# TritonDataCenter/containerpilot

Hardware: NVIDIA H100
Metric: events/sec through Bus.Publish (deliveries/s = 32-byte records landed in subscriber mailboxes) (higher is better)
Workload: dtype u8

## Files before the change

### containerpilot_b200/csrc/cpbus.cu

```cuda
#include "cpbus_internal.hpp"

#include <algorithm>
#include <chrono>
#include <cstdio>
#include <cstdlib>
#include <cstring>
#include <functional>
#include <mutex>
#include <new>
#include <string>
#include <thread>
#include <unordered_map>
#include <vector>

int cpbus_host::dev_guard(cpbus* b) {
  CK(cudaSetDevice(b->device));
  return CPBUS_OK;
}

static std::chrono::microseconds stream_budget(const cpbus* b) {
  return std::chrono::microseconds(b->stream_spin_us ? b->stream_spin_us : 2000000u);
}

static int stream_error(const cpbus* b) {
// ... 30 lines not shown
    if (f->dbg_head == -1) break;
    const cpbus_event e = f->dbg[f->dbg_tail % 10];
    if (f->dbg_tail == f->dbg_head) { f->dbg_head = -1; f->dbg_tail = 0; }
    else f->dbg_tail = (f->dbg_tail + 1) % 10;
    if (e.code == CPBUS_NONE && e.source_id == 0) break;
    if (k < cap) out[k] = e;
    k++;
  }
  return k;
}

void cpbus_host::dbg_mark_device_batch(HostFront* f, unsigned long long launch) {
  f->dbg_pending.push_back(DbgItem{true, launch, cpbus_event{}});
  if (f->dbg_pending.size() > (size_t)kAcctDbgRing) f->dbg_pending.pop_front();
}

static int rebuild_order(cpbus* b) {
  std::vector<uint32_t> order;
  static_assert(sizeof(b->h_active[0]) == 1, "h_active is a byte vector");
  mask_order(b->h_mask.data(), reinterpret_cast<const uint8_t*>(b->h_active.data()), b->n_next, b->R, b->order_block, true, order);
  b->n_order = (uint32_t)order.size();
  if (b->n_order) {
    CK(cudaMemcpyAsync(b->d_order, order.data(), (size_t)b->n_order * 4, cudaMemcpyHostToDevice, b->stream));
    CK(cudaStreamSynchronize(b->stream));
  }
  b->order_dirty = false;
  return CPBUS_OK;
}

constexpr int kFanoutMaxSmem = 200 * 1024;

enum { kLaunchPlain = 0, kLaunchFollow = 1, kLaunchRound = 2 };

template <int STORE, bool TIMERS, bool DIGEST, bool ORDERED, bool PAIRS = false>
static int launch_fanout_t(cpbus* b, const FanoutParams& p, uint32_t grid, size_t smem, int kind) {
  static bool attr_done[3][64] = {};
  void (*kernel)(FanoutParams) = kind == kLaunchRound  ? fanout_round_kernel<STORE, TIMERS, DIGEST, ORDERED, PAIRS>
                               : kind == kLaunchFollow ? fanout_follow_kernel<STORE, TIMERS, DIGEST, ORDERED, PAIRS>
                                                       : fanout_kernel<STORE, TIMERS, DIGEST, ORDERED, PAIRS>;
  const int dev = b->device & 63;
  if (!attr_done[kind][dev]) {
    CK(cudaFuncSetAttribute(kernel, cudaFuncAttributeMaxDynamicSharedMemorySize, kFanoutMaxSmem));
    attr_done[kind][dev] = true;
  }
  cudaLaunchConfig_t cfg{};
  cfg.gridDim = dim3(grid); cfg.blockDim = dim3(kThreads); cfg.dynamicSmemBytes = smem; cfg.stream = b->stream;
  cudaLaunchAttribute attr[1];
  attr[0].id = cudaLaunchAttributeProgrammaticStreamSerialization;
  attr[0].val.programmaticStreamSerializationAllowed = 1;
  cfg.attrs = attr; cfg.numAttrs = b->pdl && kind != kLaunchRound ? 1 : 0;
  CK(cudaLaunchKernelEx(&cfg, kernel, p));
  CK(cudaGetLastError());
  return CPBUS_OK;
}

template <int ST>
static int preload_round_fanouts() {
  void (*ks[])(FanoutParams) = {
      fanout_round_kernel<ST, false, false, false>, fanout_round_kernel<ST, false, true, false>,
      fanout_round_kernel<ST, true, false, false>, fanout_round_kernel<ST, true, true, false>,
      fanout_round_kernel<ST, false, false, true>, fanout_round_kernel<ST, false, true, true>,
      fanout_round_kernel<ST, true, false, false, true>, fanout_round_kernel<ST, true, true, false, true>};
  for (auto k : ks) CK(cudaFuncSetAttribute(k, cudaFuncAttributeMaxDynamicSharedMemorySize, kFanoutMaxSmem));
  return CPBUS_OK;
}

static int preload_round_kernels(cpbus* b) {
  static bool done[64] = {};
  static std::mutex mu;
  std::lock_guard<std::mutex> g(mu);
  if (done[b->device & 63]) return CPBUS_OK;
  int rc;
  if ((rc = preload_round_fanouts<CPBUS_STORE_V4>()) || (rc = preload_round_fanouts<CPBUS_STORE_V8>()) ||
      (rc = preload_round_fanouts<CPBUS_STORE_BULK>()))
    return rc;
  cudaFuncAttributes a;
  CK(cudaFuncGetAttributes(&a, stream_round_decide_kernel));
  CK(cudaFuncGetAttributes(&a, stream_round_admit_kernel));
  CK(cudaFuncGetAttributes(&a, stream_round_agree_kernel));
  CK(cudaFuncGetAttributes(&a, consume_all_kernel));
  CK(cudaFuncGetAttributes(&a, digest_fold_kernel));
  CK(cudaFuncGetAttributes(&a, blockers_scan_kernel));
  CK(cudaFuncGetAttributes(&a, lagging_scan_kernel));
  done[b->device & 63] = true;
  return CPBUS_OK;
}

struct StreamArgs {
  const StreamHdr* hdr = nullptr; unsigned long long* ack = nullptr; unsigned long long seq = 0;
  const StreamHdr* next_hdr = nullptr;
  uint32_t off = 0; bool final = true;
  FollowRec* follow_rec = nullptr;
  bool follow_from_host = false;
  const RoundDev* round = nullptr;
};
// ... 23 lines not shown
  if (n == 0 && b->n_timers == 0 && !sa) return CPBUS_OK;
  FanoutParams p{};
  p.batch = d_src; p.ring = b->d_ring; p.ctl = b->d_ctl; p.timers = b->d_timers; p.stats = b->d_stats; p.pow_table = b->d_pow; p.launch_seq = ++b->launch_seq;
  p.desc = b->d_desc + (p.launch_seq & 1) * ((fanout_desc_bytes(2048) + 255) & ~(size_t)255);
  p.desc_ready = b->d_desc_ready + (p.launch_seq & 1) * 16; p.w_now = w;
  p.result = result_slot(b, p.launch_seq); p.result_next = result_slot(b, p.launch_seq + 1);
  p.batch_local = b->d_batch_local; p.staged = (uint32_t)o.staged;
  p.err_word = b->h_err.dev(); p.acct = o.account ? b->d_acct.get() : nullptr;
  p.pf_state = b->d_pf_state; p.pf_buf = b->d_pf_buf; p.pf_stride = b->B; p.spin_us = b->stream_spin_us;
  if (sa) {
    p.stream_hdr = sa->hdr; p.stream_ack = sa->ack; p.stream_seq = sa->seq; p.stream_next_hdr = sa->next_hdr;
    p.stream_off = sa->off; p.stream_final = sa->final ? 1u : 0u;
  }
  const bool follow = sa && sa->follow_rec, round = sa && sa->round;
  const int kind = round ? kLaunchRound : follow ? kLaunchFollow : kLaunchPlain;
  p.round = round ? sa->round : nullptr;
  if (follow) {
    p.follow_clock = b->d_follow_clock; p.follow_rec = sa->follow_rec; p.follow_window = max_window(b);
    p.follow_from_host = sa->follow_from_host ? 1u : 0u;
  }
  p.prefetch_src = o.pf_src; p.prefetch_dst = o.pf_dst; p.prefetch_n = o.pf_n;
  p.batch_dep = o.batch_dep ? 1u : 0u; p.n_ev = n;
  p.n_subs = b->n_next; p.ring_cap = b->R; p.K = b->K; p.sub_base = b->cfg.sub_id_base;
  p.use_digest = b->use_digest; p.lossless = b->lossless; p.timers_on = b->n_timers > 0 && b->K > 0;
  p.smem_cap = (n + 31u) & ~31u;
  const size_t hot_bytes = (size_t)b->n_next * (sizeof(SubCtl) + (p.timers_on ? b->K * sizeof(DevTimer) : 0));
  p.hints = b->hints >= 0 ? (uint32_t)b->hints : (hot_bytes <= (64u << 20) ? 1u : 0u);
  const uint32_t need = (b->n_next + kWarpsPerCta - 1) / kWarpsPerCta;
  uint32_t grid = b->cfg.grid_ctas ? std::max(1u, std::min(b->cfg.grid_ctas, need)) : 0u;
  int rc;
  const bool pairs_on = b->n_paired > 0 && b->d_pairs;
  p.pairs = pairs_on ? b->d_pairs.get() : nullptr;
  size_t smem = fanout_smem_bytes(p.smem_cap) + (pairs_on ? kPairFilterBytes : 0);
  if (!pairs_on && !p.timers_on && b->n_filtered > 0) {
    if (b->order_dirty) { const int rc_order = rebuild_order(b); if (rc_order) return rc_order; }
    if (b->n_order) {
      const uint32_t scale = std::max(1u, (p.n_ev + 128u) / 256u);
      uint32_t spw = b->subs_per_warp ? std::min(32u, b->subs_per_warp)
                                      : std::max(4u, std::min(16u / scale, b->n_order / (20480u * scale)));
      p.order = b->d_order; p.n_order = b->n_order; p.spw = spw;
      const uint32_t warps = (b->n_order + spw - 1) / spw;
      grid = std::max(1u, (warps + kWarpsPerCta - 1) / kWarpsPerCta);
    }
  }
  if (pairs_on && !b->cfg.grid_ctas) {
    const uint32_t blocks = (b->n_next + 31u) / 32u;
    grid = std::max(1u, std::min((blocks + kWarpsPerCta - 1) / kWarpsPerCta, (uint32_t)b->sm_count * 16u));
  }
  if (!pairs_on && !p.order) {
    uint32_t spw = b->subs_per_warp;
    if (grid) spw = std::max(1u, (need + grid - 1) / grid);
    else if (!spw) {
      const uint32_t scale = std::max(1u, (p.n_ev + 128u) / 256u);
      const uint32_t cap = std::max(1u, 16u / scale);
      spw = std::max(1u, std::min(cap, (need + (uint32_t)b->sm_count * 7 * scale) / ((uint32_t)b->sm_count * 14 * scale)));
    }
    p.spw = spw;
    grid = std::max(1u, (need + spw - 1) / spw);
    const size_t off = fanout_stage_off(p.smem_cap);
    const size_t per_sub = sizeof(SubCtl) + (p.timers_on ? (size_t)b->K * sizeof(DevTimer) : 0);
    const size_t min_round = (size_t)kWarpsPerCta * per_sub;
    const size_t ctas = std::max<size_t>(1, std::min<size_t>(kCtasPerSm, b->smem_per_sm / (off + min_round + b->smem_reserved)));
    const size_t room = std::min<size_t>(kFanoutMaxSmem, b->smem_per_sm / ctas - b->smem_reserved) - off;
    p.stage_subs = std::max<uint32_t>(kWarpsPerCta, (uint32_t)std::min<size_t>((size_t)kWarpsPerCta * spw, room / per_sub) & ~7u);
    smem = off + p.stage_subs * per_sub;
  }
  const int variant = pairs_on ? (p.use_digest ? 7 : 6) : (p.timers_on ? 2 : 0) | (p.use_digest ? 1 : 0) | (p.order ? 4 : 0);
  std::unique_lock<std::mutex> ready_lock(b->mu, std::defer_lock);
  if (b->sparse_drains) ready_lock.lock();
#define CPBUS_DISPATCH(ST)                                                              \
  switch (variant) {                                                                     \
    case 0: rc = launch_fanout_t<ST, false, false, false>(b, p, grid, smem, kind); break;      \
    case 1: rc = launch_fanout_t<ST, false, true, false>(b, p, grid, smem, kind); break;       \
    case 2: rc = launch_fanout_t<ST, true, false, false>(b, p, grid, smem, kind); break;       \
    case 3: rc = launch_fanout_t<ST, true, true, false>(b, p, grid, smem, kind); break;        \
    case 4: rc = launch_fanout_t<ST, false, false, true>(b, p, grid, smem, kind); break;       \
    case 5: rc = launch_fanout_t<ST, false, true, true>(b, p, grid, smem, kind); break;        \
    case 6: rc = launch_fanout_t<ST, true, false, false, true>(b, p, grid, smem, kind); break; \
    default: rc = launch_fanout_t<ST, true, true, false, true>(b, p, grid, smem, kind); break; \
  }
  switch (b->store) {
    case CPBUS_STORE_V4: CPBUS_DISPATCH(CPBUS_STORE_V4); break;
    case CPBUS_STORE_BULK: CPBUS_DISPATCH(CPBUS_STORE_BULK); break;
    default: CPBUS_DISPATCH(CPBUS_STORE_V8); break;
  }
#undef CPBUS_DISPATCH
  if (b->sparse_drains) b->ready_ix.full();
  if (rc) return rc;
  b->st.kernel_launches++;
  if (!round) b->st.batches++;
  if (sa) return CPBUS_OK;
  launched_to(b, w);
  if (o.account && n) dbg_mark_device_batch(b, p.launch_seq);
  return CPBUS_OK;
}

static void timer_table(cpbus* b) {
  b->h_timers.resize((size_t)b->N * b->K);
  if (b->sparse) b->due.init(b->h_timers.size());
}

static int stage_batch(cpbus* b, uint32_t n, cpbus_event** d_dst) {
  const uint32_t slot = b->dev_slot;
  *d_dst = b->d_stage + (size_t)slot * b->B;
  if (slot % cpbus::kDevEpoch == 0) CK(cudaEventSynchronize(b->epoch_done[slot / cpbus::kDevEpoch]));
  if (n) {
    CK(cudaMemcpyAsync(*d_dst, b->h_batch[b->cur], (size_t)n * sizeof(cpbus_event), cudaMemcpyHostToDevice, b->copy_stream));
    CK(cudaEventRecord(b->h2d_done[b->cur], b->copy_stream));
  }
  return CPBUS_OK;
}

// ... 268 lines not shown
  if ((uint64_t)cfg->sub_id_base + cfg->n_max_subs > CPBUS_TARGET_ALL) return CPBUS_EINVAL;
  *R_out = R; *B_out = B;
  return CPBUS_OK;
}

int cpbus_create(const cpbus_config* cfg, cpbus_t** out) try {
  if (!cfg || !out) return CPBUS_EINVAL;
  *out = nullptr;
  uint32_t R = 0, B = 0;
  if (config_check(cfg, &R, &B)) return CPBUS_EINVAL;
  if ((cfg->flags & CPBUS_CFG_SPARSE_RECORDS) && !(cfg->flags & CPBUS_CFG_SPARSE_TICKS)) return CPBUS_EINVAL;
  if ((cfg->flags & CPBUS_CFG_SPARSE_DRAINS) && !(cfg->flags & CPBUS_CFG_SPARSE_TICKS)) return CPBUS_EINVAL;
  const uint32_t K = cfg->timers_per_sub;
  int ndev = 0;
  if (cudaGetDeviceCount(&ndev) != cudaSuccess || ndev == 0) {
    snprintf(g_cuda_err, sizeof(g_cuda_err), "no CUDA device visible");
    return CPBUS_ENODEV;
  }
  cpbus* b = new (std::nothrow) cpbus();
  if (!b) return CPBUS_ENOMEM;
  b->cfg = *cfg; b->cfg.ring_cap = R; b->cfg.batch_cap = B;
  b->N = cfg->n_max_subs; b->R = R; b->B = B; b->K = K;
  b->lossless = cfg->flags & CPBUS_CFG_LOSSLESS; b->use_digest = cfg->flags & CPBUS_CFG_DIGEST;
  b->sparse = cfg->flags & CPBUS_CFG_SPARSE_TICKS;
  b->sparse_records = cfg->flags & CPBUS_CFG_SPARSE_RECORDS;
  b->sparse_drains = cfg->flags & CPBUS_CFG_SPARSE_DRAINS;
  b->drop_missed = cfg->flags & CPBUS_CFG_DROP_MISSED_TICKS;
  b->room_lb = R;
  b->store = cfg->store_path == CPBUS_STORE_AUTO ? CPBUS_STORE_V8 : (int)cfg->store_path;
  if (const char* e = getenv("CPBUS_PDL")) b->pdl = atoi(e) != 0;
  if (const char* e = getenv("CPBUS_HINTS")) b->hints = atoi(e);
  if (const char* e = getenv("CPBUS_SUBS_PER_WARP")) b->subs_per_warp = (uint32_t)atoi(e);
  if (const char* e = getenv("CPBUS_ORDER_BLOCK")) b->order_block = (uint32_t)atoll(e);
  int rc = CPBUS_OK;
  auto fail = [&](int code) { cpbus_destroy(b); return code; };
  if (cfg->device >= 0) b->device = cfg->device;
  else if (cudaGetDevice(&b->device) != cudaSuccess) return fail(CPBUS_ECUDA);
  if (b->device >= ndev) return fail(CPBUS_EINVAL);
  if ((rc = dev_guard(b))) return fail(rc);
  cudaDeviceProp prop{};
  if (cudaGetDeviceProperties(&prop, b->device) == cudaSuccess) {
    b->sm_count = prop.multiProcessorCount;
    b->smem_per_sm = prop.sharedMemPerMultiprocessor; b->smem_reserved = prop.reservedSharedMemPerBlock;
  }
  if (cfg->stream) b->stream = (cudaStream_t)cfg->stream;
  else {
    if (cudaStreamCreateWithFlags(&b->stream, cudaStreamNonBlocking) != cudaSuccess) return fail(CPBUS_ECUDA);
    b->own_stream = true;
  }
  const size_t N = b->N;
  auto alloc = [](auto& buf, size_t n) {
    if (buf.alloc(n) == cudaSuccess) return true;
    snprintf(g_cuda_err, sizeof(g_cuda_err), "cudaMalloc(%zu) failed", n * sizeof(*buf.get()));
    return false;
  };
  if (!alloc(b->d_ring, N * R) || !alloc(b->d_ctl, N) || !alloc(b->d_order, N) || (K && !alloc(b->d_timers, N * K)) ||
      !alloc(b->d_stats, 1) || !alloc(b->d_fold, 4 * cpbus::kFoldSlots) || !alloc(b->d_pow, kPowTableLen) ||
      !alloc(b->d_desc, 2 * ((fanout_desc_bytes(2048) + 255) & ~(size_t)255)) || !alloc(b->d_desc_ready, 32))
    return fail(CPBUS_ENOMEM);
  if (cudaMemsetAsync(b->d_desc_ready, 0, 256, b->stream) != cudaSuccess) return fail(CPBUS_ECUDA);
  if (b->copy_stream.create() != cudaSuccess || b->result_stream.create() != cudaSuccess || b->launched.create() != cudaSuccess)
    return fail(CPBUS_ECUDA);
  if (b->sparse && (b->plan_done.create() != cudaSuccess || b->records_done.create() != cudaSuccess)) return fail(CPBUS_ECUDA);
  if (!alloc(b->d_stage, (size_t)cpbus::kDevSlots * B)) return fail(CPBUS_ENOMEM);
  for (CudaEvent& e : b->epoch_done) if (e.create() != cudaSuccess) return fail(CPBUS_ECUDA);
  for (int i = 0; i < cpbus::kStage; i++) {
// ... 1889 lines not shown
```

### containerpilot_b200/csrc/cpbus_fanout_body.cuh

```cuda
  constexpr bool STAGED = !ORDERED && !PAIRS;
  extern __shared__ __align__(128) unsigned char smem[];
  const uint32_t cap = p.smem_cap;
  cpbus_event* s_batch = reinterpret_cast<cpbus_event*>(smem);
  uint64_t* s_rhash = reinterpret_cast<uint64_t*>(smem + (size_t)cap * 32);
  uint2* s_meta = reinterpret_cast<uint2*>(smem + (size_t)cap * 40);
  uint64_t* s_q = reinterpret_cast<uint64_t*>(smem + (size_t)cap * 48);
  uint32_t* s_dsum = reinterpret_cast<uint32_t*>(s_q + cap + 2);
  uint32_t* s_present = s_dsum + 40;
  uint64_t* s_pow = s_q + cap + 2 + 20 + (PAIRS ? kPairFilterWords / 2 : 0);
  BatchSummary* s_sum = reinterpret_cast<BatchSummary*>(s_pow + cap + 66);
  uint32_t* s_tick = reinterpret_cast<uint32_t*>(s_sum + 1);
  const uint4* s_ctl4 = reinterpret_cast<const uint4*>(smem + fanout_stage_off(cap));
  const uint4* s_tim4 = s_ctl4 + 2u * p.stage_subs;

  const int tid = threadIdx.x, lane = tid & 31, warp = tid >> 5;
  uint32_t n = FOLLOW ? 0u : p.n_ev;
  uint64_t w_follow = 0;
  unsigned long long round_ack = 0;

  if (p.batch_dep) asm volatile("griddepcontrol.wait;" ::: "memory");
  const bool stream = p.staged == 2u;
  const uint32_t pf_slot = stream ? (uint32_t)(p.stream_seq % kStreamPrefetch) : 0u;
  uint32_t pos = ORDERED ? (blockIdx.x * kWarpsPerCta + warp) * p.spw : 0u;
  uint32_t my_ids = 0;
  if (ORDERED && pos + lane < min(pos + p.spw, p.n_order)) my_ids = __ldg(p.order + pos + lane);
  if (tid == 0) {
    mbar_init(&s_sum->mbar, 1); mbar_init(&s_sum->mbar_desc, 1); mbar_init(&s_sum->mbar_state, 1);
    s_sum->acc_deliv = 0; s_sum->acc_ticks = 0; s_sum->acc_dig_lo = 0; s_sum->acc_dig_hi = 0;
    s_sum->stream_local = (stream && !p.lossless && p.stream_off == 0 && __ldcg(p.pf_state + pf_slot) == p.stream_seq) ? 1u : 0u;
    s_sum->own_desc = blockIdx.x == 0 ? 1u : 0u; s_sum->abort_launch = 0;
  }
  __syncthreads();
  const bool stream_local = stream && s_sum->stream_local;
  const bool staged = FOLLOW || (p.staged && !stream_local);
  const cpbus_event* batch_src = stream_local ? p.pf_buf + (size_t)pf_slot * p.pf_stride : p.batch;
  if (tid == 0) {
    const uint32_t pow_bytes = ((cap + 65u) * 8u + 15u) & ~15u;
    const bool direct = n && !staged;
    mbar_expect_tx(&s_sum->mbar, (direct ? n * 32u : 0u) + pow_bytes);
    if (direct) bulk_g2s(s_batch, batch_src, n * 32u, &s_sum->mbar);
    bulk_g2s(s_pow, p.pow_table, pow_bytes, &s_sum->mbar);
  }

  const bool keep = p.hints & 1u;

  const uint32_t desc_bytes = 24u * cap + 16u + 160u + (PAIRS ? kPairFilterBytes : 0u);
// ... 205 lines not shown
  } else {
    mbar_wait(&s_sum->mbar_desc, 0);
    if constexpr (FOLLOW) {
      n = s_sum->abort_launch ? 0u : s_dsum[kFollowN];
      w_follow = ((uint64_t)s_dsum[kFollowWHi] << 32) | s_dsum[kFollowWLo];
    }
    mbar_wait(&s_sum->mbar, (staged && n && !s_sum->abort_launch) ? 1u : 0u);
  }
  constexpr bool PLANAR = STORE != CPBUS_STORE_BULK && !ORDERED;
  const uint32_t hi_off = cap;
  if (PLANAR && n) {
    uint4* sq = reinterpret_cast<uint4*>(s_batch);
    uint4 v[8];
    __syncthreads();
#pragma unroll
    for (int r = 0; r < 8; r++) { const uint32_t q = tid + r * kThreads; if (q < 2u * n) v[r] = sq[q]; }
    __syncthreads();
#pragma unroll
    for (int r = 0; r < 8; r++) { const uint32_t q = tid + r * kThreads; if (q < 2u * n) sq[(q & 1u) * hi_off + (q >> 1)] = v[r]; }
    __syncthreads();
  }
  auto ev_ts = [&](uint32_t i) -> uint64_t {
    return PLANAR ? reinterpret_cast<const uint64_t*>(reinterpret_cast<const uint4*>(s_batch) + i)[1] : s_batch[i].ts_ns;
  };
  auto ev_code_src = [&](uint32_t i) -> uint2 {
    return PLANAR ? reinterpret_cast<const uint2*>(reinterpret_cast<const uint4*>(s_batch) + hi_off + i)[0] : make_uint2(s_batch[i].code, s_batch[i].source_id);
  };
  const bool aborted = s_sum->abort_launch != 0;
  const uint32_t K = p.K, J = K ? 32u / K : 32u;
  const uint32_t tk_slot = lane / J, tk_j = lane % J;
  const bool timers_on = TIMERS && p.timers_on && K;
  const uint32_t wstride = gridDim.x * kWarpsPerCta;
  uint32_t pos_end = (aborted || !ORDERED) ? 0u : min(pos + p.spw, p.n_order);
  const uint32_t pos_step = ORDERED ? 1u : kWarpsPerCta;
  const uint32_t pos0 = pos;
  uint32_t s = ORDERED ? __shfl_sync(0xffffffffu, my_ids, 0) : pos;
  if (!p.batch_dep) asm volatile("griddepcontrol.wait;" ::: "memory");
  asm volatile("griddepcontrol.launch_dependents;");
  const uint32_t rng_first = blockIdx.x * kWarpsPerCta * p.spw, rng_end = min(rng_first + kWarpsPerCta * p.spw, p.n_subs);
  auto stage_round = [&](uint32_t first) {
    if (!STAGED || tid != 0 || aborted || first >= rng_end) return;
    const uint32_t rn = min(p.stage_subs, rng_end - first);
    asm volatile("fence.proxy.async.shared::cta;" ::: "memory");
    const uint32_t tim_bytes = timers_on ? rn * K * (uint32_t)sizeof(DevTimer) : 0u;
    mbar_expect_tx(&s_sum->mbar_state, rn * (uint32_t)sizeof(SubCtl) + tim_bytes);
    bulk_g2s_hint(const_cast<uint4*>(s_ctl4), p.ctl + first, rn * (uint32_t)sizeof(SubCtl), &s_sum->mbar_state, keep);
    if (tim_bytes) bulk_g2s_hint(const_cast<uint4*>(s_tim4), p.timers + (size_t)first * K, tim_bytes, &s_sum->mbar_state, keep);
  };
  uint4 ca = make_uint4(0, 0, 0, 0), cb = ca, ta = ca;
  if (ORDERED && pos < pos_end) ld_sector(p.ctl + s, ca, cb, keep);
  const uint32_t present = s_dsum[0];
  const bool has_unicast = s_dsum[1] != 0;
  bool bulk_pending = false;
  uint32_t tri_blk = blockIdx.x * kWarpsPerCta + warp, tri_base = 0, tri_live = 0;
  uint4 tri_a = make_uint4(0, 0, 0, 0), tri_b = tri_a;
  uint32_t rnd_first = rng_first, rnd_phase = 0;
  for (;;) {
  if constexpr (STAGED) {
    if (aborted || rnd_first >= rng_end) break;
    stage_round(rnd_first);
    mbar_wait(&s_sum->mbar_state, rnd_phase);
    rnd_phase ^= 1u;
    pos = rnd_first + warp; pos_end = rnd_first + min(p.stage_subs, rng_end - rnd_first);
  }
  if constexpr (PAIRS) {
    bool exhausted = aborted;
    while (!tri_live && !exhausted) {
      tri_base = tri_blk * 32u;
      if (tri_base >= p.n_subs) { exhausted = true; break; }
      tri_blk += wstride;
      const uint32_t sl = tri_base + lane;
      bool live = false;
      tri_a = make_uint4(0, 0, 0, 0); tri_b = tri_a;
      if (sl < p.n_subs) ld_sector(p.ctl + sl, tri_a, tri_b, keep);
      const uint32_t ml = tri_b.z;
      if (ml & kActiveBit) {
        live = has_unicast || (ml & present) != 0;
        if (!live && timers_on) {
          const uint32_t nsl = min((ml >> kTimerHintShift) & 0xFu, K);
          for (uint32_t t = 0; t < nsl && !live; t++) {
            uint4 h;
            ld_half(p.timers + (size_t)sl * K + t, h, keep);
            const uint64_t due = ((uint64_t)h.y << 32) | h.x;
            live = due != kTimerIdle && due <= (FOLLOW ? w_follow : p.w_now);
          }
        }
        if (!live && (ml & kPairBit)) {
          const uint4* row = reinterpret_cast<const uint4*>(p.pairs + (size_t)sl * CPBUS_MAX_PAIRS);
          for (uint32_t q = 0; q < CPBUS_MAX_PAIRS / 2 && !live; q++) {
            const uint4 v = __ldg(row + q);
            if (v.x >= 32u) break;
            uint32_t h = pair_key_hash(v.x, v.y);
            live = ((s_present[(h & 32767u) >> 5] >> (h & 31u)) & (s_present[((h >> 15) & 32767u) >> 5] >> ((h >> 15) & 31u)) & 1u) != 0;
            if (live || v.z >= 32u) { if (!live) break; continue; }
            h = pair_key_hash(v.z, v.w);
            live = ((s_present[(h & 32767u) >> 5] >> (h & 31u)) & (s_present[((h >> 15) & 32767u) >> 5] >> ((h >> 15) & 31u)) & 1u) != 0;
          }
        }
      }
      tri_live = __ballot_sync(0xffffffffu, live);
    }
    if (exhausted) break;
    const uint32_t jl = (uint32_t)__ffs(tri_live) - 1u;
    tri_live &= tri_live - 1u;
    pos = tri_base + jl; pos_end = pos + 1u; s = pos;
    ca = make_uint4(__shfl_sync(0xffffffffu, tri_a.x, jl), __shfl_sync(0xffffffffu, tri_a.y, jl), __shfl_sync(0xffffffffu, tri_a.z, jl), __shfl_sync(0xffffffffu, tri_a.w, jl));
    cb = make_uint4(__shfl_sync(0xffffffffu, tri_b.x, jl), __shfl_sync(0xffffffffu, tri_b.y, jl), __shfl_sync(0xffffffffu, tri_b.z, jl), __shfl_sync(0xffffffffu, tri_b.w, jl));
    if (timers_on && tk_slot < K) ld_half(p.timers + (size_t)s * K + tk_slot, ta, keep);
  }
  const uint32_t Rm = p.ring_cap - 1;
  const uint4* s4 = reinterpret_cast<const uint4*>(s_batch);
  const uint32_t scratch_words = max(32u, cap / 2u);
  uint32_t* my_tick = s_tick + warp * scratch_words;

  uint32_t run_mask = 0xffffffffu, run_k = 0;
  uint64_t run_sum = 0;
  for (; pos < pos_end; pos += pos_step) {
    const uint32_t si = pos - rnd_first;
    uint4 cur_a = ca, cur_b = cb;
    auto ctl_half = [&](uint32_t h) -> uint4 { return STAGED ? s_ctl4[2u * si + h] : (h ? cur_b : cur_a); };
    auto tim_half = [&](uint32_t h) -> uint4 {
      if (STAGED) return s_tim4[2u * (si * K + tk_slot) + h];
      if (!h) return ta;
      uint4 cold;
      ld_half(reinterpret_cast<const unsigned char*>(p.timers + (size_t)s * K + tk_slot) + 16, cold, keep);
      return cold;
    };
    if (STAGED) { cur_a = ctl_half(0); cur_b = ctl_half(1); }
    if (ORDERED) s = __shfl_sync(0xffffffffu, my_ids, (pos - pos0) & 31); else s = pos;
    if (ORDERED) {
      const uint32_t pn = pos + pos_step;
      if (pn < pos_end) ld_sector(p.ctl + __shfl_sync(0xffffffffu, my_ids, (pn - pos0) & 31), ca, cb, keep);
    }
    const uint32_t m = cur_b.z;
    if (!(m & kActiveBit)) continue;
    const uint64_t tail = ((uint64_t)cur_a.y << 32) | cur_a.x;
    cpbus_event* ring = p.ring + (size_t)s * p.ring_cap;
    const uint32_t gid = p.sub_base + s;
    const uint32_t nslots = timers_on ? min((m >> kTimerHintShift) & 0xFu, K) : 0u;
    const bool dense = !has_unicast && ((m & present) == present);

    uint32_t n_ticks = 0, tk_mask = 0, tk_rank = 0, tk_src = 0, tk_fired = 0;
    bool tk_valid = false; uint64_t tk_due = 0, tk_period = 0;
    if (nslots) {
      uint64_t tk_due0 = kTimerIdle;
      if (TIMERS && tk_slot < nslots) {
        const uint4 hot = tim_half(0);
        tk_due0 = ((uint64_t)hot.y << 32) | hot.x; tk_period = ((uint64_t)hot.w << 32) | hot.z;
      }
      const uint64_t step = (uint64_t)tk_j * tk_period;
      tk_due = tk_due0 + step;
      const bool wraps = __umul64hi(tk_j, tk_period) != 0 || tk_due < step || tk_due == kTimerIdle;
      tk_valid = tk_due0 != kTimerIdle && !wraps && tk_due <= (FOLLOW ? w_follow : p.w_now) && (tk_j == 0 || tk_period != 0);
      tk_mask = __ballot_sync(0xffffffffu, tk_valid);
      n_ticks = __popc(tk_mask);
      if (n_ticks) {

        if (J == 32 || (tk_mask >> J) == 0) tk_rank = tk_j;
        else {
#pragma unroll 1
          for (int t = 0; t < 32; t++) {
            if (!((tk_mask >> t) & 1u)) continue;
// ... 80 lines not shown
      for (; c0 + 64 <= n; c0 += 64) {
        const uint32_t o0 = slot_of(c0), o1 = slot_of(c0 + 32);
        copy_record_pairs<PLANAR>(s4, hi_off, ring, (uint32_t)tail, Rm, c0 + lane, o0, true);
        copy_record_pairs<PLANAR>(s4, hi_off, ring, (uint32_t)tail, Rm, c0 + 32 + lane, o1, true);
      }
#pragma unroll 1
      for (; c0 < n; c0 += 32) {
        const uint32_t out = slot_of(c0);
        copy_record_pairs<PLANAR>(s4, hi_off, ring, (uint32_t)tail, Rm, c0 + lane, out, c0 + lane < n);
      }
      if (!cold_early && TIMERS && tk_slot < nslots) {
        const uint4 cold = tim_half(1);
        tk_src = cold.x; tk_fired = cold.y;
      }
      if (tk_valid) {
        const uint32_t out = tk_pos + tk_rank;
        const uint64_t w0 = (uint64_t)tk_fired + tk_j, w1 = tk_due;
        const uint64_t w2 = (uint64_t)CPBUS_TIMER_EXPIRED | ((uint64_t)tk_src << 32);
        const uint64_t w3 = (uint64_t)gid | ((uint64_t)CPBUS_F_TICK << 32);
        const uint4 a = make_uint4((uint32_t)w0, (uint32_t)(w0 >> 32), (uint32_t)w1, (uint32_t)(w1 >> 32));
        const uint4 b = make_uint4((uint32_t)w2, (uint32_t)(w2 >> 32), (uint32_t)w3, (uint32_t)(w3 >> 32));
        st_v8(ring + (((uint32_t)tail + out) & Rm), a, b);
        if (DIGEST) {
          const uint32_t prev = tk_rank ? my_tick[tk_rank - 1] : 0u;
          dsum = (s_q[tk_pos] - s_q[prev]) * s_pow[n_ticks - tk_rank] + record_hash_words(w0, w1, w2, w3) * s_pow[k - 1 - out];
          if (tk_rank == n_ticks - 1) dsum += s_q[n] - s_q[tk_pos];
        }
      }
      if (DIGEST) dsum = warp_sum64(dsum);
      __syncwarp();
    } else if (!(PAIRS && pair_live) && !has_unicast && n_ticks == 0) {
      if constexpr (!TIMERS) {
        uint16_t* my_idx = reinterpret_cast<uint16_t*>(my_tick);
        const bool reuse = ORDERED && (m & CPBUS_MASK_ALL) == run_mask;
        if (!reuse) {
          uint32_t base = 0;
          const uint32_t nchunks = (n + 31) >> 5;
          for (uint32_t c0 = 0; c0 < nchunks; c0 += 4) {
            uint32_t cbit[4];
#pragma unroll
            for (uint32_t u = 0; u < 4; u++) {
              const uint32_t i = (c0 + u) * 32 + lane;
              cbit[u] = i < n ? s_meta[i].x : 0u;
            }
#pragma unroll
            for (uint32_t u = 0; u < 4; u++) {
              const bool match = (m & cbit[u]) != 0;
              const uint32_t w = __ballot_sync(0xffffffffu, match);
              if (match) my_idx[base + __popc(w & ((1u << lane) - 1u))] = (uint16_t)((c0 + u) * 32 + lane);
              base += __popc(w);
            }
          }
          run_k = base;
          __syncwarp();
        }
        k = run_k;
        uint64_t acc = 0;
        const uint64_t p32 = s_pow[32];
        const bool hashing = DIGEST && !reuse;
        uint32_t i0 = (uint32_t)lane < k ? my_idx[lane] : 0u, i1 = lane + 32u < k ? my_idx[lane + 32] : 0u;
        for (uint32_t o0 = 0; o0 < k; o0 += 64) {
          const uint32_t o = o0 + lane;
          const bool v0 = o < k, v1 = o + 32 < k;
          const uint32_t n0 = o + 64 < k ? my_idx[o + 64] : 0u, n1 = o + 96 < k ? my_idx[o + 96] : 0u;
          copy_record_pairs<PLANAR>(s4, hi_off, ring, (uint32_t)tail, Rm, i0, o, v0);
          copy_record_pairs<PLANAR>(s4, hi_off, ring, (uint32_t)tail, Rm, i1, o + 32, v1);
          if (hashing) {
            if (v0) acc = acc * p32 + s_rhash[i0];
            if (v1) acc = acc * p32 + s_rhash[i1];
          }
          i0 = n0; i1 = n1;
        }
        if (DIGEST) {
          if (reuse) dsum = run_sum;
          else {
            const uint32_t cnt = k > (uint32_t)lane ? (k - lane + 31u) / 32u : 0u;
            dsum = cnt ? acc * s_pow[k - 1 - (lane + 32u * (cnt - 1u))] : 0ull;
            dsum = warp_sum64(dsum);
            if (ORDERED) run_sum = dsum;
          }
        }
        if (ORDERED) run_mask = m & CPBUS_MASK_ALL;
        __syncwarp();
      } else {
        uint32_t kk = ((m >> lane) & 1u) ? s_dsum[2 + lane] : 0u;
        kk = __reduce_add_sync(0xffffffffu, kk);
        k = kk;
        uint32_t base = 0;
        const uint32_t nchunks = (n + 31) >> 5;
        for (uint32_t c = 0; c < nchunks; c++) {
          const uint32_t i = c * 32 + lane;
          const bool match = i < n && (m & s_meta[i].x) != 0;
          const uint32_t w = __ballot_sync(0xffffffffu, match);
          const uint32_t out = base + __popc(w & ((1u << lane) - 1u));
          if (DIGEST && match) dsum += s_rhash[i] * s_pow[k - 1 - out];
          copy_record_pairs<PLANAR>(s4, hi_off, ring, (uint32_t)tail, Rm, i, out, match);
          base += __popc(w);
        }
        if (DIGEST) dsum = warp_sum64(dsum);
      }
    } else {
      const uint32_t nchunks = (n + 31) >> 5;
      uint2 my_pair = make_uint2(kPairNone, 0u);
      uint32_t n_pairs = 0, pair_codes = 0;
      if (PAIRS && pair_live) {
        if (lane < CPBUS_MAX_PAIRS) my_pair = __ldg(p.pairs + (size_t)s * CPBUS_MAX_PAIRS + lane);
        const bool used = my_pair.x < 32u;
        n_pairs = __popc(__ballot_sync(0xffffffffu, used));
        pair_codes = __reduce_or_sync(0xffffffffu, used ? (1u << my_pair.x) : 0u);
      }
      uint32_t myword = 0;
      for (uint32_t c = 0; c < nchunks; c++) {
        const uint32_t i = c * 32 + lane;
        bool match = false, cand = false;
        if (i < n) {
// ... 184 lines not shown
```

### containerpilot_b200/csrc/cpbus_internal.hpp

```cpp
#pragma once
#include <cstdio>
#include <deque>
#include <mutex>
#include <new>
#include <string>
#include <unordered_map>
#include <vector>

#include "../../include/cpbus.h"
#include "cpbus_kernels.cuh"
#include "cuda_owned.hpp"
#include "host_index.hpp"

using namespace cpbus_dev;
using namespace cuda_owned;

#define CK(call)                                                                                   \
  do {                                                                                             \
    cudaError_t e_ = (call);                                                                       \
    if (e_ != cudaSuccess) {                                                                       \
      snprintf(g_cuda_err, sizeof(g_cuda_err), "%s:%d %s: %s", __FILE__, __LINE__, #call,          \
               cudaGetErrorString(e_));                                                            \
      return CPBUS_ECUDA;                                                                          \
    }                                                                                              \
// ... 95 lines not shown
  MappedBuf<RoundRec> h_round;
  DeviceBuf<RoundDev> d_round;
  MappedBuf<FollowRec> h_follow;
  DeviceBuf<unsigned long long> d_follow_clock;
  int follow_next = 0;
  CudaEvent follow_done;
  std::recursive_mutex follow_mu;
  DeviceBuf<DevPubAcct> d_acct;
  PinnedBuf<unsigned char> h_acct;
  DevPubAcct* host_acct() const { return reinterpret_cast<DevPubAcct*>(h_acct.get()); }
  DeviceBuf<cpbus_event> d_drain;
  DeviceBuf<uint2> d_drain_idx;
  DeviceBuf<unsigned long long> d_ready_lb;
  DeviceBuf<cpbus_ready> d_ready; DeviceBuf<uint32_t> d_ready_slot;
  MappedBuf<unsigned long long> h_ready_hdr;
  static constexpr int kDrainTickets = 8;
  struct DrainTicket {
    MappedBuf<unsigned char> buf;
    CudaEvent done;
    bool busy = false;
    uint32_t ticket = 0, first = 0, n = 0, start = 0;
    size_t cap = 0, ready_cap = 0;
    uint64_t place = 0;
    bool take = false, whole = false, none = false;
  };
  DrainTicket drain_tk[kDrainTickets];
  uint32_t drain_tk_gen = 0, drain_tk_busy = 0;
  DeviceBuf<unsigned long long> d_lag_lb;
  MappedBuf<unsigned long long> h_lag_hdr;
  MappedBuf<uint32_t> h_block;
  MappedBuf<cpbus_lag> h_lag;
  uint32_t subs_per_warp = 0;
  uint32_t order_block = 0;
  bool pdl = true;
  CudaEvent launched;
  int hints = -1;
  static constexpr int kFoldSlots = 8;
  DeviceBuf<unsigned long long> d_fold;
  CudaEvent fold_done[kFoldSlots];
  uint32_t fold_next = 0;
  static constexpr int kStage = 8;
  static constexpr int kDevSlots = 64, kDevEpoch = 16;
  DeviceBuf<cpbus_event> d_stage;
  CudaEvent epoch_done[kDevSlots / kDevEpoch];
  uint32_t dev_slot = 0;
  PinnedBuf<cpbus_event> h_batch[kStage];
  CudaEvent h2d_done[kStage];
  CudaStream copy_stream;
  CudaStream result_stream;
  DeviceBuf<DevResultSlot> d_result;
  PinnedBuf<DevResultSlot> h_result;
  CudaEvent result_done[8];
  uint32_t result_next = 0;
  PinnedBuf<DevStats> h_stats;
  PinnedBuf<unsigned long long> h_fold;
  int cur = 0;

  std::vector<uint32_t> h_mask;
  std::vector<uint8_t> h_active;
  std::vector<uint8_t> h_npairs;
  DeviceBuf<uint2> d_pairs;
  uint32_t n_paired = 0;
  DeviceBuf<uint32_t> d_order;
  uint32_t n_order = 0, n_filtered = 0;
  bool order_dirty = true;
  uint32_t n_next = 0, n_active = 0;
// ... 152 lines not shown
```

### containerpilot_b200/csrc/cpbus_kernels.cuh

```cuda
#pragma once
#include <cstdint>
#include <cuda_runtime.h>

#include "../../include/cpbus.h"

namespace cpbus_dev {

constexpr int kWarpsPerCta = 8;
constexpr int kThreads = kWarpsPerCta * 32;
constexpr int kCtasPerSm = 4;
constexpr uint32_t kActiveBit = 0x80000000u;
constexpr int kTimerHintShift = 24;
constexpr uint32_t kPairBit = 0x10000000u;
constexpr uint32_t kPairNone = 0xFFFFFFFFu;
constexpr uint32_t kCodeOutOfRange = CPBUS_N_CODES;
static_assert(kCodeOutOfRange < (uint32_t)kTimerHintShift,"the out-of-range bit must lie between the code mask and the mask word's bookkeeping bits");
constexpr uint32_t kPairFilterWords = 1024;
constexpr uint32_t kPairFilterBytes = kPairFilterWords * 4;
__host__ __device__ inline uint32_t pair_key_hash(uint32_t code, uint32_t source_id) {
  uint32_t x = (source_id ^ (code << 27)) * 0x9E3779B1u;
  x ^= x >> 15; x *= 0x85EBCA77u; x ^= x >> 13;
  return x;
}
constexpr uint64_t kDigestP = 0x9E3779B97F4A7C15ull;
// ... 285 lines not shown
__device__ __forceinline__ void mbar_wait(uint64_t* mbar, uint32_t parity) {
  asm volatile(
      "{\n\t.reg .pred p;\n\t"
      "CPBUS_WAIT:\n\t"
      "mbarrier.try_wait.parity.shared::cta.b64 p, [%0], %1;\n\t"
      "@p bra CPBUS_DONE;\n\t"
      "bra CPBUS_WAIT;\n\t"
      "CPBUS_DONE:\n\t}" ::"r"(smem_u32(mbar)),
      "r"(parity)
      : "memory");
}

struct BatchSummary {
  uint64_t mbar;
  uint64_t mbar_desc;
  uint64_t mbar_state;
  uint32_t acc_deliv, acc_ticks, acc_pad[2];
  uint32_t acc_dig_lo, acc_dig_hi;
  uint32_t stream_local;
  uint32_t own_desc;
  uint32_t abort_launch;
  uint32_t pf_ok;
  uint64_t red[kWarpsPerCta];
};

__host__ __device__ inline size_t fanout_desc_bytes(uint32_t cap) { return (size_t)24 * cap + 16 + 160 + kPairFilterBytes; }

__host__ __device__ inline size_t fanout_smem_bytes(uint32_t cap) {
  const size_t scratch = (cap / 2u > 32u ? cap / 2u : 32u) * sizeof(uint32_t);
  return (size_t)cap * 56 + 16 + 160 + (size_t)(cap + 66) * 8 + sizeof(BatchSummary) + kWarpsPerCta * scratch + 128;
}
__host__ __device__ inline size_t fanout_stage_off(uint32_t cap) { return (fanout_smem_bytes(cap) + 127) & ~(size_t)127; }

template <int STORE, bool TIMERS, bool DIGEST, bool ORDERED, bool PAIRS = false>
__global__ void __launch_bounds__(kThreads, kCtasPerSm) fanout_kernel(const FanoutParams p) {
  constexpr bool FOLLOW = false, ROUND = false;
#include "cpbus_fanout_body.cuh"
}
template <int STORE, bool TIMERS, bool DIGEST, bool ORDERED, bool PAIRS = false>
__global__ void __launch_bounds__(kThreads, kCtasPerSm) fanout_follow_kernel(const FanoutParams p) {
  constexpr bool FOLLOW = true, ROUND = false;
#include "cpbus_fanout_body.cuh"
}
template <int STORE, bool TIMERS, bool DIGEST, bool ORDERED, bool PAIRS = false>
__global__ void __launch_bounds__(kThreads, kCtasPerSm) fanout_round_kernel(const FanoutParams p) {
  constexpr bool FOLLOW = true, ROUND = true;
#include "cpbus_fanout_body.cuh"
}

__device__ __forceinline__ void admit_body(const cpbus_event* batch, uint32_t n_ev, uint64_t w_now, const SubCtl* ctl,
                                           const DevTimer* timers, uint32_t n_subs, uint32_t ring_cap, uint32_t K,
                                           uint32_t sub_base, uint32_t timers_on, DevStats* stats, const uint2* pairs) {
  __shared__ uint32_t hist[32];
  __shared__ uint32_t s_uni;
  __shared__ unsigned long long s_max;
  if (threadIdx.x < 32) hist[threadIdx.x] = 0;
  if (threadIdx.x == 0) { s_uni = 0; s_max = 0; }
  __syncthreads();
  for (uint32_t i = threadIdx.x; i < n_ev; i += blockDim.x) {
    const uint32_t code = batch[i].code, target = batch[i].target;
    if (target == CPBUS_TARGET_ALL) { if (code < 32) atomicAdd(&hist[code], 1u); }
    else atomicAdd(&s_uni, 1u);
  }
  __syncthreads();
  const uint32_t s = blockIdx.x * blockDim.x + threadIdx.x;
  SubCtl c{};
  if (s < n_subs) c = ctl[s];
  const uint32_t m = c.mask;
  if (s < n_subs && (m & kActiveBit)) {
    uint64_t k = 0;
    for (uint32_t cc = 0; cc < CPBUS_N_CODES; cc++) if ((m >> cc) & 1u) k += hist[cc];
    if (pairs && (m & kPairBit)) {
      const uint2* my = pairs + (size_t)s * CPBUS_MAX_PAIRS;
      for (uint32_t i = 0; i < n_ev; i++) {
        const uint32_t code = batch[i].code;
        if (batch[i].target != CPBUS_TARGET_ALL || code >= CPBUS_N_CODES || ((m >> code) & 1u)) continue;
        const uint32_t src = batch[i].source_id;
// ... 929 lines not shown
```

Before: 93.12 billion.

## Sort staged subscribers by mask in shared memory to reuse per-mask fanout work

For filtered subscribers without timers or pairs, the host-built global order is replaced by a default path that ranks each staged round of subscriber control words by mask inside shared memory. Each warp then walks a contiguous slice of that sorted permutation, so consecutive subscribers with equal masks reuse the computed index list and digest. This avoids the host-side order rebuild and its synchronous copy. The trade-offs are a quadratic rank sort per round, an extra barrier, extra shared memory per subscriber, and a lower subs-per-warp cap on the non-sorted path. The old order path stays available behind CPBUS_MASK_WALK.

```diff
diff --git a/containerpilot_b200/csrc/cpbus.cu b/containerpilot_b200/csrc/cpbus.cu
--- a/containerpilot_b200/csrc/cpbus.cu
+++ b/containerpilot_b200/csrc/cpbus.cu
@@ -86,12 +86,12 @@
 
 enum { kLaunchPlain = 0, kLaunchFollow = 1, kLaunchRound = 2 };
 
-template <int STORE, bool TIMERS, bool DIGEST, bool ORDERED, bool PAIRS = false>
+template <int STORE, bool TIMERS, bool DIGEST, bool ORDERED, bool PAIRS = false, bool SORTED = false>
 static int launch_fanout_t(cpbus* b, const FanoutParams& p, uint32_t grid, size_t smem, int kind) {
   static bool attr_done[3][64] = {};
-  void (*kernel)(FanoutParams) = kind == kLaunchRound  ? fanout_round_kernel<STORE, TIMERS, DIGEST, ORDERED, PAIRS>
-                               : kind == kLaunchFollow ? fanout_follow_kernel<STORE, TIMERS, DIGEST, ORDERED, PAIRS>
-                                                       : fanout_kernel<STORE, TIMERS, DIGEST, ORDERED, PAIRS>;
+  void (*kernel)(FanoutParams) = kind == kLaunchRound  ? fanout_round_kernel<STORE, TIMERS, DIGEST, ORDERED, PAIRS, SORTED>
+                               : kind == kLaunchFollow ? fanout_follow_kernel<STORE, TIMERS, DIGEST, ORDERED, PAIRS, SORTED>
+                                                       : fanout_kernel<STORE, TIMERS, DIGEST, ORDERED, PAIRS, SORTED>;
   const int dev = b->device & 63;
   if (!attr_done[kind][dev]) {
     CK(cudaFuncSetAttribute(kernel, cudaFuncAttributeMaxDynamicSharedMemorySize, kFanoutMaxSmem));
@@ -114,7 +114,8 @@
       fanout_round_kernel<ST, false, false, false>, fanout_round_kernel<ST, false, true, false>,
       fanout_round_kernel<ST, true, false, false>, fanout_round_kernel<ST, true, true, false>,
       fanout_round_kernel<ST, false, false, true>, fanout_round_kernel<ST, false, true, true>,
-      fanout_round_kernel<ST, true, false, false, true>, fanout_round_kernel<ST, true, true, false, true>};
+      fanout_round_kernel<ST, true, false, false, true>, fanout_round_kernel<ST, true, true, false, true>,
+      fanout_round_kernel<ST, false, false, false, false, true>, fanout_round_kernel<ST, false, true, false, false, true>};
   for (auto k : ks) CK(cudaFuncSetAttribute(k, cudaFuncAttributeMaxDynamicSharedMemorySize, kFanoutMaxSmem));
   return CPBUS_OK;
 }
@@ -204,7 +205,9 @@
   const bool pairs_on = b->n_paired > 0 && b->d_pairs;
   p.pairs = pairs_on ? b->d_pairs.get() : nullptr;
   size_t smem = fanout_smem_bytes(p.smem_cap) + (pairs_on ? kPairFilterBytes : 0);
-  if (!pairs_on && !p.timers_on && b->n_filtered > 0) {
+  const bool filtered = !pairs_on && !p.timers_on && b->n_filtered > 0;
+  const bool sorted = filtered && !b->mask_walk;
+  if (filtered && b->mask_walk) {
     if (b->order_dirty) { const int rc_order = rebuild_order(b); if (rc_order) return rc_order; }
     if (b->n_order) {
       const uint32_t scale = std::max(1u, (p.n_ev + 128u) / 256u);
@@ -224,20 +227,22 @@
     if (grid) spw = std::max(1u, (need + grid - 1) / grid);
     else if (!spw) {
       const uint32_t scale = std::max(1u, (p.n_ev + 128u) / 256u);
-      const uint32_t cap = std::max(1u, 16u / scale);
+      const uint32_t cap = std::max(1u, (sorted ? 16u : 4u) / scale);
       spw = std::max(1u, std::min(cap, (need + (uint32_t)b->sm_count * 7 * scale) / ((uint32_t)b->sm_count * 14 * scale)));
     }
     p.spw = spw;
     grid = std::max(1u, (need + spw - 1) / spw);
     const size_t off = fanout_stage_off(p.smem_cap);
-    const size_t per_sub = sizeof(SubCtl) + (p.timers_on ? (size_t)b->K * sizeof(DevTimer) : 0);
+    const size_t per_sub = sizeof(SubCtl) + (p.timers_on ? (size_t)b->K * sizeof(DevTimer) : 0) + (sorted ? sizeof(uint32_t) : 0);
     const size_t min_round = (size_t)kWarpsPerCta * per_sub;
     const size_t ctas = std::max<size_t>(1, std::min<size_t>(kCtasPerSm, b->smem_per_sm / (off + min_round + b->smem_reserved)));
     const size_t room = std::min<size_t>(kFanoutMaxSmem, b->smem_per_sm / ctas - b->smem_reserved) - off;
     p.stage_subs = std::max<uint32_t>(kWarpsPerCta, (uint32_t)std::min<size_t>((size_t)kWarpsPerCta * spw, room / per_sub) & ~7u);
+    if (sorted) p.stage_subs = std::min<uint32_t>(p.stage_subs, kThreads);
     smem = off + p.stage_subs * per_sub;
   }
-  const int variant = pairs_on ? (p.use_digest ? 7 : 6) : (p.timers_on ? 2 : 0) | (p.use_digest ? 1 : 0) | (p.order ? 4 : 0);
+  const int variant = pairs_on ? (p.use_digest ? 7 : 6) : sorted ? (p.use_digest ? 9 : 8)
+                                                       : (p.timers_on ? 2 : 0) | (p.use_digest ? 1 : 0) | (p.order ? 4 : 0);
   std::unique_lock<std::mutex> ready_lock(b->mu, std::defer_lock);
   if (b->sparse_drains) ready_lock.lock();
 #define CPBUS_DISPATCH(ST)                                                              \
@@ -249,7 +254,9 @@
     case 4: rc = launch_fanout_t<ST, false, false, true>(b, p, grid, smem, kind); break;       \
     case 5: rc = launch_fanout_t<ST, false, true, true>(b, p, grid, smem, kind); break;        \
     case 6: rc = launch_fanout_t<ST, true, false, false, true>(b, p, grid, smem, kind); break; \
-    default: rc = launch_fanout_t<ST, true, true, false, true>(b, p, grid, smem, kind); break; \
+    case 7: rc = launch_fanout_t<ST, true, true, false, true>(b, p, grid, smem, kind); break;  \
+    case 8: rc = launch_fanout_t<ST, false, false, false, false, true>(b, p, grid, smem, kind); break; \
+    default: rc = launch_fanout_t<ST, false, true, false, false, true>(b, p, grid, smem, kind); break; \
   }
   switch (b->store) {
     case CPBUS_STORE_V4: CPBUS_DISPATCH(CPBUS_STORE_V4); break;
@@ -584,6 +591,7 @@
   if (const char* e = getenv("CPBUS_HINTS")) b->hints = atoi(e);
   if (const char* e = getenv("CPBUS_SUBS_PER_WARP")) b->subs_per_warp = (uint32_t)atoi(e);
   if (const char* e = getenv("CPBUS_ORDER_BLOCK")) b->order_block = (uint32_t)atoll(e);
+  if (const char* e = getenv("CPBUS_MASK_WALK")) b->mask_walk = atoi(e) != 0;
   int rc = CPBUS_OK;
   auto fail = [&](int code) { cpbus_destroy(b); return code; };
   if (cfg->device >= 0) b->device = cfg->device;
diff --git a/containerpilot_b200/csrc/cpbus_fanout_body.cuh b/containerpilot_b200/csrc/cpbus_fanout_body.cuh
--- a/containerpilot_b200/csrc/cpbus_fanout_body.cuh
+++ b/containerpilot_b200/csrc/cpbus_fanout_body.cuh
@@ -1,4 +1,6 @@
   constexpr bool STAGED = !ORDERED && !PAIRS;
+  static_assert(!SORTED || (STAGED && !TIMERS), "SORTED: the staged build without timers");
+  constexpr bool REUSE = ORDERED || SORTED;
   extern __shared__ __align__(128) unsigned char smem[];
   const uint32_t cap = p.smem_cap;
   cpbus_event* s_batch = reinterpret_cast<cpbus_event*>(smem);
@@ -12,6 +14,7 @@
   uint32_t* s_tick = reinterpret_cast<uint32_t*>(s_sum + 1);
   const uint4* s_ctl4 = reinterpret_cast<const uint4*>(smem + fanout_stage_off(cap));
   const uint4* s_tim4 = s_ctl4 + 2u * p.stage_subs;
+  uint32_t* s_perm = reinterpret_cast<uint32_t*>(smem + fanout_stage_off(cap)) + 8u * p.stage_subs;
 
   const int tid = threadIdx.x, lane = tid & 31, warp = tid >> 5;
   uint32_t n = FOLLOW ? 0u : p.n_ev;
@@ -283,7 +286,7 @@
   const bool timers_on = TIMERS && p.timers_on && K;
   const uint32_t wstride = gridDim.x * kWarpsPerCta;
   uint32_t pos_end = (aborted || !ORDERED) ? 0u : min(pos + p.spw, p.n_order);
-  const uint32_t pos_step = ORDERED ? 1u : kWarpsPerCta;
+  const uint32_t pos_step = REUSE ? 1u : kWarpsPerCta;
   const uint32_t pos0 = pos;
   uint32_t s = ORDERED ? __shfl_sync(0xffffffffu, my_ids, 0) : pos;
   if (!p.batch_dep) asm volatile("griddepcontrol.wait;" ::: "memory");
@@ -313,6 +316,21 @@
     mbar_wait(&s_sum->mbar_state, rnd_phase);
     rnd_phase ^= 1u;
     pos = rnd_first + warp; pos_end = rnd_first + min(p.stage_subs, rng_end - rnd_first);
+    if constexpr (SORTED) {
+      const uint32_t rn = pos_end - rnd_first;
+      for (uint32_t t = tid; t < rn; t += kThreads) {
+        const uint32_t key = s_ctl4[2u * t + 1u].z & CPBUS_MASK_ALL;
+        uint32_t rank = 0;
+        for (uint32_t j = 0; j < rn; j++) {
+          const uint32_t kj = s_ctl4[2u * j + 1u].z & CPBUS_MASK_ALL;
+          rank += (kj < key || (kj == key && j < t)) ? 1u : 0u;
+        }
+        s_perm[rank] = t;
+      }
+      __syncthreads();
+      const uint32_t share = (rn + kWarpsPerCta - 1) / kWarpsPerCta;
+      pos = rnd_first + min(rn, warp * share); pos_end = rnd_first + min(rn, (warp + 1) * share);
+    }
   }
   if constexpr (PAIRS) {
     bool exhausted = aborted;
@@ -367,7 +385,7 @@
   uint32_t run_mask = 0xffffffffu, run_k = 0;
   uint64_t run_sum = 0;
   for (; pos < pos_end; pos += pos_step) {
-    const uint32_t si = pos - rnd_first;
+    const uint32_t si = SORTED ? s_perm[pos - rnd_first] : pos - rnd_first;
     uint4 cur_a = ca, cur_b = cb;
     auto ctl_half = [&](uint32_t h) -> uint4 { return STAGED ? s_ctl4[2u * si + h] : (h ? cur_b : cur_a); };
     auto tim_half = [&](uint32_t h) -> uint4 {
@@ -378,7 +396,7 @@
       return cold;
     };
     if (STAGED) { cur_a = ctl_half(0); cur_b = ctl_half(1); }
-    if (ORDERED) s = __shfl_sync(0xffffffffu, my_ids, (pos - pos0) & 31); else s = pos;
+    if (ORDERED) s = __shfl_sync(0xffffffffu, my_ids, (pos - pos0) & 31); else s = SORTED ? rnd_first + si : pos;
     if (ORDERED) {
       const uint32_t pn = pos + pos_step;
       if (pn < pos_end) ld_sector(p.ctl + __shfl_sync(0xffffffffu, my_ids, (pn - pos0) & 31), ca, cb, keep);
@@ -525,7 +543,7 @@
     } else if (!(PAIRS && pair_live) && !has_unicast && n_ticks == 0) {
       if constexpr (!TIMERS) {
         uint16_t* my_idx = reinterpret_cast<uint16_t*>(my_tick);
-        const bool reuse = ORDERED && (m & CPBUS_MASK_ALL) == run_mask;
+        const bool reuse = REUSE && (m & CPBUS_MASK_ALL) == run_mask;
         if (!reuse) {
           uint32_t base = 0;
           const uint32_t nchunks = (n + 31) >> 5;
@@ -570,10 +588,10 @@
             const uint32_t cnt = k > (uint32_t)lane ? (k - lane + 31u) / 32u : 0u;
             dsum = cnt ? acc * s_pow[k - 1 - (lane + 32u * (cnt - 1u))] : 0ull;
             dsum = warp_sum64(dsum);
-            if (ORDERED) run_sum = dsum;
-          }
-        }
-        if (ORDERED) run_mask = m & CPBUS_MASK_ALL;
+            if (REUSE) run_sum = dsum;
+          }
+        }
+        if (REUSE) run_mask = m & CPBUS_MASK_ALL;
         __syncwarp();
       } else {
         uint32_t kk = ((m >> lane) & 1u) ? s_dsum[2 + lane] : 0u;
diff --git a/containerpilot_b200/csrc/cpbus_internal.hpp b/containerpilot_b200/csrc/cpbus_internal.hpp
--- a/containerpilot_b200/csrc/cpbus_internal.hpp
+++ b/containerpilot_b200/csrc/cpbus_internal.hpp
@@ -151,6 +151,7 @@
   MappedBuf<cpbus_lag> h_lag;
   uint32_t subs_per_warp = 0;
   uint32_t order_block = 0;
+  bool mask_walk = false;
   bool pdl = true;
   CudaEvent launched;
   int hints = -1;
diff --git a/containerpilot_b200/csrc/cpbus_kernels.cuh b/containerpilot_b200/csrc/cpbus_kernels.cuh
--- a/containerpilot_b200/csrc/cpbus_kernels.cuh
+++ b/containerpilot_b200/csrc/cpbus_kernels.cuh
@@ -341,17 +341,17 @@
 }
 __host__ __device__ inline size_t fanout_stage_off(uint32_t cap) { return (fanout_smem_bytes(cap) + 127) & ~(size_t)127; }
 
-template <int STORE, bool TIMERS, bool DIGEST, bool ORDERED, bool PAIRS = false>
+template <int STORE, bool TIMERS, bool DIGEST, bool ORDERED, bool PAIRS = false, bool SORTED = false>
 __global__ void __launch_bounds__(kThreads, kCtasPerSm) fanout_kernel(const FanoutParams p) {
   constexpr bool FOLLOW = false, ROUND = false;
 #include "cpbus_fanout_body.cuh"
 }
-template <int STORE, bool TIMERS, bool DIGEST, bool ORDERED, bool PAIRS = false>
+template <int STORE, bool TIMERS, bool DIGEST, bool ORDERED, bool PAIRS = false, bool SORTED = false>
 __global__ void __launch_bounds__(kThreads, kCtasPerSm) fanout_follow_kernel(const FanoutParams p) {
   constexpr bool FOLLOW = true, ROUND = false;
 #include "cpbus_fanout_body.cuh"
 }
-template <int STORE, bool TIMERS, bool DIGEST, bool ORDERED, bool PAIRS = false>
+template <int STORE, bool TIMERS, bool DIGEST, bool ORDERED, bool PAIRS = false, bool SORTED = false>
 __global__ void __launch_bounds__(kThreads, kCtasPerSm) fanout_round_kernel(const FanoutParams p) {
   constexpr bool FOLLOW = true, ROUND = true;
 #include "cpbus_fanout_body.cuh"
```

Measured after the change: 94.06 billion, median of 6. +1.0%, better.
